# congliuUvA/Clifford-Group-Equivariant-Simplicial-Message-Passing-Networks

Measured on AMD Instinct MI355X. Metric: simplicial edges/sec (fwd+bwd) on Cl(3,0) 8-ch multivectors; % HBM roofline, higher is better.
Workload: dtype f32; 1 GPU; S1: EGCL layer fwd+bwd, Cl(1, 1, 1), 8 channels, 10000 nodes, 100000 edges/GPU x 1 GPU, aggr=mean, edge_attr 6ch, node_attr 3ch; aggregation=float atomics, launch=hip-graph replay

## Files before the change

clifford-group-equivariant-simplicial-message-passing-networks_amd/csmpn_hip/native.py:

```python
from __future__ import annotations

import ctypes as C
import os

_HERE = os.path.dirname(os.path.abspath(__file__))
LIB_PATH = os.environ.get("CSMPN_LIB") or os.path.join(_HERE, "libcsmpn_hip.so")

ABI_VERSION = 2
MAX_BLOCKS = 4
FLAG_WEIGHTS_PACKED = 1
FLAG_NO_VALIDATE = 2
FLAG_DETERMINISTIC = 4
FLAG_SAVE_STATE = 8
ERR_UNSUPPORTED, ERR_INVALID, ERR_HIP = 1, 2, 3

EXPORTS = (
    "csmpn_metric_supported",
    "csmpn_algebra_tables",
    "csmpn_geometric_product_forward",
    "csmpn_geometric_product_backward",
    "csmpn_cemlp_workspace_bytes",
    "csmpn_cemlp_saved_floats_per_row",
    "csmpn_cemlp_saved_floats",
    "csmpn_cemlp_forward",
# ... 4 lines not shown
    "csmpn_mvsilu_backward",
    "csmpn_mvnorm_forward",
    "csmpn_mvnorm_backward",
    "csmpn_mvlayernorm_forward",
    "csmpn_mvlayernorm_backward",
    "csmpn_wgp_forward",
    "csmpn_wgp_backward",
    "csmpn_csr_workspace_bytes",
    "csmpn_csr_build",
    "csmpn_csr_source_order",
    "csmpn_segment_reduce",
    "csmpn_egcl_edge_forward",
    "csmpn_egcl_edge_backward",
    "csmpn_egcl_node_forward",
    "csmpn_egcl_node_backward",
    "csmpn_simplex_rows",
    "csmpn_embed_cemlp_forward",
    "csmpn_embed_cemlp_backward",
    "csmpn_type_attr_forward",
    "csmpn_type_attr_backward",
    "csmpn_readout_mse_forward",
    "csmpn_readout_mse_backward",
    "csmpn_readout_traj_forward",
    "csmpn_readout_traj_backward",
    "csmpn_last_error",
    "csmpn_last_kernel",
    "csmpn_abi_version",
    "csmpn_build_target",
)

# ... 61 lines not shown
    sig("csmpn_mvlayernorm_backward", C.c_int, [fp, C.c_int, vp, vp, vp, i64, i32, vp, vp, vp])
    sig("csmpn_wgp_forward", C.c_int, [fp, C.c_int, vp, vp, vp, i64, i32, vp, vp])
    sig("csmpn_wgp_backward", C.c_int, [fp, C.c_int, vp, vp, vp, vp, i64, i32, vp, vp, vp, vp])
    sig("csmpn_csr_workspace_bytes", sz, [i64, i64])
    sig("csmpn_csr_build", C.c_int, [vp, i64, i64, vp, vp, vp, vp, vp, vp, sz, u32, vp])
    sig("csmpn_csr_source_order", C.c_int, [vp, i64, i64, vp, vp, vp, sz, vp])
    sig("csmpn_segment_reduce", C.c_int, [vp, i64, i64, vp, vp, vp, vp, vp, i32, vp])
    sig("csmpn_egcl_edge_forward", C.c_int,
        [fp, C.c_int, bp, C.c_int, vp, i32, vp, i32, vp, vp, vp, i64, i64, vp, vp, vp, sz, u32, vp])
    sig("csmpn_egcl_edge_backward", C.c_int,
        [fp, C.c_int, bp, bg, C.c_int, vp, i32, vp, i32, vp, vp, vp, i64, i64, vp, vp, vp, vp, vp, sz, u32, vp])
    sig("csmpn_egcl_node_forward", C.c_int,
        [fp, C.c_int, bp, C.c_int, vp, i32, vp, i32, vp, i32, vp, i32, i32, i64, vp, vp, vp, sz, u32, vp])
    sig("csmpn_egcl_node_backward", C.c_int,
        [fp, C.c_int, bp, bg, C.c_int, vp, i32, vp, i32, vp, i32, vp, i32, i32, i64, vp, vp, vp, vp, vp, vp, sz, u32, vp])
    sig("csmpn_simplex_rows", C.c_int, [C.c_int, C.POINTER(VertexBlock), C.c_int, vp, i64, i32, i64, vp, vp])
    sig("csmpn_embed_cemlp_forward", C.c_int, [fp, C.c_int, bp, C.c_int, vp, i64, i32, vp, i32, i32, i64, vp, vp, vp, sz, u32, vp])
    sig("csmpn_embed_cemlp_backward", C.c_int, [fp, C.c_int, bp, bg, C.c_int, vp, i64, i32, vp, i32, i32, i64, vp, vp, vp, sz, u32, vp])
    sig("csmpn_type_attr_forward", C.c_int, [C.c_int, vp, i32, i32, vp, i64, vp, vp, i64, vp, vp, vp])
    sig("csmpn_type_attr_backward", C.c_int, [C.c_int, i32, i32, vp, i64, vp, vp, i64, vp, vp, vp, vp])
    sig("csmpn_readout_mse_forward", C.c_int, [C.c_int, vp, vp, i32, vp, i64, i32, vp, i64, vp, vp, vp, vp, vp])
    sig("csmpn_readout_mse_backward", C.c_int, [C.c_int, vp, i32, i64, i32, vp, i64, vp, vp, vp])
    sig("csmpn_readout_traj_forward", C.c_int, [C.c_int, vp, i32, vp, i64, vp, i32, i32, vp, vp, vp, vp, i64, vp, vp, vp, vp])
    sig("csmpn_readout_traj_backward", C.c_int,
        [C.c_int, vp, i32, i64, vp, vp, i64, vp, i32, i32, vp, vp, vp, vp, vp, vp, vp, vp, vp, vp, vp])
    sig("csmpn_last_error", C.c_char_p, [])
    sig("csmpn_last_kernel", C.c_char_p, [])
    sig("csmpn_abi_version", C.c_int, [])
    sig("csmpn_build_target", C.c_char_p, [])
    return lib
# ... 25 lines not shown
```

clifford-group-equivariant-simplicial-message-passing-networks_amd/csmpn_hip/ops.py:

```python
from __future__ import annotations

import ctypes as C
import os
import warnings
from typing import List, Optional, Sequence

import torch

from . import native
from .native import BlockGrads, BlockParams, PARAM_FIELDS, check

NP = len(PARAM_FIELDS)


def _stream(device) -> int:
    return torch.cuda.current_stream(device).cuda_stream


def _on_device_of(arg_index):
    import functools

    def deco(fn):
        @functools.wraps(fn)
        def wrapped(*args, **kwargs):
# ... 505 lines not shown
            rc = native.lib().csmpn_egcl_edge_backward(
                e.metric_arr, e.n, e.params, e.grads, e.nblk, h.data_ptr(), spec.C, _ptr(edge_attr), spec.A,
                csr.perm.data_ptr(), csr.src.data_ptr(), csr.dst.data_ptr(), csr.n_edges, N, g_agg.data_ptr(),
                rows.data_ptr(), _ptr(g_ea), _ptr(saved), ws.data_ptr(), ws.numel(),
                flags | native.FLAG_DETERMINISTIC, _stream(dev))
            if not (det == "soft" and _soft_fallback(rc)):
                check(rc)
                segment_reduce(rows, gh, add=(csr.row_ptr, None), sub=csr.source_order())
                return g_ea, views
        check(native.lib().csmpn_egcl_edge_backward(
            e.metric_arr, e.n, e.params, e.grads, e.nblk, h.data_ptr(), spec.C, _ptr(edge_attr), spec.A,
            csr.perm.data_ptr(), csr.src.data_ptr(), csr.dst.data_ptr(), csr.n_edges, N, g_agg.data_ptr(),
            gh.data_ptr(), _ptr(g_ea), _ptr(saved), ws.data_ptr(), ws.numel(), flags, _stream(dev)))
        return g_ea, views


_SAVE_STATE = os.environ.get("CSMPN_SAVE_STATE", "1") not in ("0", "")


def _check_egcl_inputs(spec, csr, h, edge_attr, node_attr, n_edges):
    D = spec.edge.D
    if h.dim() != 3 or h.shape[1] != spec.C or h.shape[2] != D:
        raise RuntimeError(f"h must be [N, {spec.C}, {D}], got {tuple(h.shape)}")
    if (edge_attr is None) != (spec.A == 0) or (node_attr is None) != (spec.T == 0):
        raise RuntimeError("edge_attr/node_attr presence does not match edge_attr_features/node_attr_features")
    if edge_attr is not None and tuple(edge_attr.shape) != (n_edges, spec.A, D):
        raise RuntimeError(f"edge_attr must be [{n_edges}, {spec.A}, {D}], got {tuple(edge_attr.shape)}")
    if node_attr is not None and tuple(node_attr.shape) != (h.shape[0], spec.T, D):
        raise RuntimeError(f"node_attr must be [{h.shape[0]}, {spec.T}, {D}], got {tuple(node_attr.shape)}")

# ... 41 lines not shown
        pos = 2
        edge_attr = node_attr = None
        if ctx.has_ea:
            edge_attr = saved[pos]; pos += 1
        if ctx.has_na:
            node_attr = saved[pos]; pos += 1
        it = iter(saved[pos:])
        params = [next(it) if m else None for m in ctx.mask]
        ne = spec.edge.nblk * NP
        pe, pn = params[:ne], params[ne:]
        gout = gout.contiguous()
        gfe, gfn = ctx.gflats if ctx.gflats is not None else (None, None)
        ctx.gflats = None
        refs = ctx.param_refs
        fuse = _fusable(refs, h.device)
        gh, g_agg, g_na, views_n = HipBackend.node_backward(spec, csr.deg, h, agg, node_attr, pn, gout,
                                                            ctx.needs_input_grad[2], ctx.st_n, gfn,
                                                            fused_into=refs[ne:] if fuse else None)
        g_ea, views_e = HipBackend.edge_backward(spec, csr, h, edge_attr, pe, g_agg, gh, ctx.needs_input_grad[1],
                                                 ctx.st_e, gfe, fused_into=refs[:ne] if fuse else None)
        return (gh, g_ea, g_na, None, None, *views_e, *views_n)


def egcl_apply(h, edge_attr, node_attr, spec: EgclSpec, csr: Csr, params):
    return _EgclFn.apply(h, edge_attr, node_attr, spec, csr, *params)




class _GpFn(torch.autograd.Function):
# ... 448 lines not shown
```

clifford-group-equivariant-simplicial-message-passing-networks_amd/csrc/capi.hip:

```cpp
#include <mutex>
#include <hip/hip_runtime.h>

#include <cstdarg>
#include <cstdio>
#include <cstdlib>
#include <cstring>
#include <vector>

#include "plan.hpp"

using namespace csmpn;

thread_local char g_csmpn_err[512] = "";

int csmpn_fail(int code, const char* fmt, ...) {
    va_list ap;
    va_start(ap, fmt);
    vsnprintf(g_csmpn_err, sizeof(g_csmpn_err), fmt, ap);
    va_end(ap);
    return code;
}


namespace csmpn {
// ... 258 lines not shown
                            float* save_inputs, void* workspace, size_t workspace_bytes, uint32_t flags, void* stream) {
    const AlgId id = alg_id(metric, n);
    if (id == ALG_NONE) return fail(CSMPN_ERR_UNSUPPORTED, "metric not supported by the HIP path");
    RowIO io;
    int rc = edge_io(blocks, h, channels, edge_attr, attr_channels, perm, src_sorted, dst_sorted, E, flags, io);
    if (rc) return rc;
    Plan plan;
    if ((rc = make_plan(id, blocks, nullptr, n_blocks, workspace, workspace_bytes, false, blocks[n_blocks - 1].out_features << n, false,
                        E, plan, (flags & CSMPN_FLAG_DETERMINISTIC) != 0))) return rc;
    const bool need_pack = !(flags & CSMPN_FLAG_WEIGHTS_PACKED);
    io.agg = agg; io.save = save_inputs;
    (void)N;
    return run_rows(plan, MODE_EDGE, false, io, (hipStream_t)stream, need_pack);
}

int csmpn_egcl_edge_backward(const float* metric, int n, const csmpn_block_params* blocks,
                             const csmpn_block_grads* grads, int n_blocks, const float* h, int32_t channels,
                             const float* edge_attr, int32_t attr_channels, const int32_t* perm,
                             const int32_t* src_sorted, const int32_t* dst_sorted, int64_t E, int64_t N,
                             const float* g_agg, float* gh, float* g_edge_attr, const float* saved_inputs, void* workspace,
                             size_t workspace_bytes, uint32_t flags, void* stream) {
    const AlgId id = alg_id(metric, n);
    if (id == ALG_NONE) return fail(CSMPN_ERR_UNSUPPORTED, "metric not supported by the HIP path");
    RowIO io;
    int rc = edge_io(blocks, h, channels, edge_attr, attr_channels, perm, src_sorted, dst_sorted, E, flags, io);
    if (rc) return rc;
    Plan plan;
    if ((rc = make_plan(id, blocks, grads, n_blocks, workspace, workspace_bytes, true, 0, saved_inputs != nullptr, E, plan,
                        (flags & CSMPN_FLAG_DETERMINISTIC) != 0))) return rc;
    const bool need_pack = true;
    io.gy = g_agg; io.gx[0] = gh; io.gx[1] = g_edge_attr; io.saved = saved_inputs;
    (void)N;
    return run_rows(plan, MODE_EDGE, true, io, (hipStream_t)stream, need_pack, (flags & CSMPN_FLAG_WEIGHTS_PACKED) != 0);
}

static int node_io(const csmpn_block_params* blocks, int n_blocks, const float* h, int channels, const float* agg,
                   int agg_channels, const float* node_attr, int attr_channels, const int32_t* in_degree,
                   int mean_aggr, int residual, int64_t N, RowIO& io) {
    if (attr_channels > 0 && !node_attr) return fail(CSMPN_ERR_INVALID, "node_attr is null");
    if (channels + agg_channels + attr_channels != blocks[0].in_features)
        return fail(CSMPN_ERR_INVALID, "node model in_features %d != %d + %d + %d", blocks[0].in_features, channels,
                    agg_channels, attr_channels);
    if (residual && blocks[n_blocks - 1].out_features != channels)
        return fail(CSMPN_ERR_INVALID, "residual needs out_features == channels");
    if (mean_aggr && !in_degree) return fail(CSMPN_ERR_INVALID, "in_degree is null");
    memset(&io, 0, sizeof(io));
    io.rows = N; io.nseg = attr_channels > 0 ? 3 : 2;
    io.seg[0].a = h; io.seg[0].ch = channels; io.seg[0].off = 0;
// ... 11 lines not shown
    if (id == ALG_NONE) return fail(CSMPN_ERR_UNSUPPORTED, "metric not supported by the HIP path");
    RowIO io;
    int rc = node_io(blocks, n_blocks, h, channels, agg, agg_channels, node_attr, attr_channels, in_degree, mean_aggr,
                     residual, N, io);
    if (rc) return rc;
    Plan plan;
    if ((rc = make_plan(id, blocks, nullptr, n_blocks, workspace, workspace_bytes, false, 0, false, N, plan,
                        (flags & CSMPN_FLAG_DETERMINISTIC) != 0))) return rc;
    const bool need_pack = !(flags & CSMPN_FLAG_WEIGHTS_PACKED);
    io.y = out; io.resid = residual ? h : nullptr; io.save = save_inputs;
    io.row_store = (flags & CSMPN_FLAG_DETERMINISTIC) ? 1 : 0;
    io.save_state = (flags & CSMPN_FLAG_SAVE_STATE) ? 1 : 0;
    return run_rows(plan, MODE_NODE, false, io, (hipStream_t)stream, need_pack);
}

int csmpn_egcl_node_backward(const float* metric, int n, const csmpn_block_params* blocks,
                             const csmpn_block_grads* grads, int n_blocks, const float* h, int32_t channels,
                             const float* agg, int32_t agg_channels, const float* node_attr, int32_t attr_channels,
                             const int32_t* in_degree, int32_t mean_aggr, int32_t residual, int64_t N,
                             const float* g_out, float* gh, float* g_agg, float* g_node_attr, const float* saved_inputs, void* workspace,
                             size_t workspace_bytes, uint32_t flags, void* stream) {
    const AlgId id = alg_id(metric, n);
    if (id == ALG_NONE) return fail(CSMPN_ERR_UNSUPPORTED, "metric not supported by the HIP path");
    RowIO io;
    int rc = node_io(blocks, n_blocks, h, channels, agg, agg_channels, node_attr, attr_channels, in_degree, mean_aggr,
                     residual, N, io);
    if (rc) return rc;
    Plan plan;
    if ((rc = make_plan(id, blocks, grads, n_blocks, workspace, workspace_bytes, true, 0, saved_inputs != nullptr, N, plan,
                        (flags & CSMPN_FLAG_DETERMINISTIC) != 0))) return rc;
    const bool need_pack = true;
    io.gy = g_out; io.gx[0] = gh; io.gx[1] = g_agg; io.gx[2] = g_node_attr;
    io.resid_bwd = residual ? 1 : 0; io.saved = saved_inputs;
    io.row_store = (flags & CSMPN_FLAG_DETERMINISTIC) ? 1 : 0;
    io.save_state = (flags & CSMPN_FLAG_SAVE_STATE) ? 1 : 0;
    return run_rows(plan, MODE_NODE, true, io, (hipStream_t)stream, need_pack, (flags & CSMPN_FLAG_WEIGHTS_PACKED) != 0);
}

}
```

clifford-group-equivariant-simplicial-message-passing-networks_amd/csrc/cemlp_cl.hpp:

```cpp
#pragma once
#include "cemlp_lane.hpp"

namespace csmpn {

constexpr int kClWaves = 4;
constexpr int kClSliceCap = 512;
constexpr int kClParStride = 36;

#define CL_LDS_ORDER() do { asm volatile("" ::: "memory"); __builtin_amdgcn_wave_barrier(); asm volatile("" ::: "memory"); } while (0)

struct ClStamp {
#ifdef CSMPN_STAMPS
    static constexpr int kSlots = 24;
    unsigned long long t0, acc[kSlots];
    CSMPN_DEV explicit ClStamp(int) {
#pragma unroll
        for (int i = 0; i < kSlots; ++i) acc[i] = 0;
        t0 = __builtin_amdgcn_s_memtime();
    }
    CSMPN_DEV void operator()(int id) {
        __builtin_amdgcn_sched_barrier(0);
        const unsigned long long t1 = __builtin_amdgcn_s_memtime();
        acc[id] += t1 - t0;
        t0 = t1;
// ... 1116 lines not shown
        ClStage<ALG, C, TB1, true> st1;
        st0.load(Cd.b[0], threadIdx.x, dir);
        if constexpr (NBLK > 1) st1.load(Cd.b[1], threadIdx.x, dir);
        st0.store(smem, threadIdx.x);
        if constexpr (NBLK > 1) st1.store(smem + TB0::total, threadIdx.x);
    }
    __syncthreads();
    stamp(0);
    const long ntiles = (io.rows + ClMap<C>::RPW - 1) / ClMap<C>::RPW;
    if (ntiles <= (long)gridDim.x * kClWaves) cl_bwd_blocks<ALG, C, MODE, NBLK, NA, SAVES, true>(io, smem, T0, req, stamp);
    else cl_bwd_blocks<ALG, C, MODE, NBLK, NA, SAVES, false>(io, smem, T0, req, stamp);
    stamp.flush(io.stamps, threadIdx.x & 63);
}

template <class ALG, int C, int I0, int NBLK>
__global__ void __launch_bounds__(256) cl_reduce_kernel(const DevCemlp Cd, const float* part, int nslices, int slice_cap) {
    constexpr int G = ALG::G;
    using P0 = ClPart<ALG, C, I0>;
    using P1 = ClPart<ALG, C, C>;
    constexpr int total = P0::total + (NBLK > 1 ? P1::total : 0);
    __shared__ float red[16][17];
    const int j = threadIdx.x & 15, w = threadIdx.x >> 4;
    int e = blockIdx.x * 16 + j;
    const bool live = e < total;
    if (!live) e = 0;
    const int k = (NBLK > 1 && e >= P0::total) ? 1 : 0;
    const int len = k == 0 ? P0::total : P1::total;
    const float* p = part + (k == 0 ? 0 : (size_t)slice_cap * P0::total);
    if (k == 1) e -= P0::total;
    float s = 0.f;
    for (int s0 = w; s0 < nslices; s0 += 256) {
        float v[16];
#pragma unroll
        for (int i = 0; i < 16; ++i) {
            const int sl = s0 + 16 * i;
            v[i] = sl < nslices ? p[(size_t)sl * len + e] : 0.f;
        }
#pragma unroll
// ... 12 lines not shown
    if (f < nW1) dst = B.gW1 + f;
    else if ((f -= nW1) < nWC) dst = B.gWR + f;
    else if ((f -= nWC) < nWC) dst = B.gWL + f;
    else {
        f -= nWC;
        if (f < P0::qsa) dst = B.has_b1 ? B.gb1 + f : nullptr;
        else if (f < P0::qsb) dst = B.gsa + (f - P0::qsa);
        else if (f < P0::qw) dst = B.gsb + (f - P0::qsb);
        else if (f < P0::qan) dst = B.gw + (f - P0::qw);
        else if (f < P0::qbL) dst = B.gan + (f - P0::qan);
        else if (f < P0::qla) dst = B.gbL + (f - P0::qbL);
        else dst = B.gla + (f - P0::qla);
    }
    if (dst) *dst += s;
}

}
```

clifford-group-equivariant-simplicial-message-passing-networks_amd/csrc/cemlp_device.hpp:

```cpp
#pragma once
#include <hip/hip_runtime.h>

#include "algebra.hpp"

namespace csmpn {

typedef float f4 __attribute__((ext_vector_type(4)));

#define CSMPN_DEV __device__ __forceinline__
#define CSMPN_PHASE() __builtin_amdgcn_sched_barrier(0)

constexpr float kInvSqrt2 = 0.70710678118654752440f;
constexpr float kEps = 1e-6f;
constexpr float kSmooth = 1e-16f;


struct DevBlock {
    int I, O;
    int KKi, KKo;
    int NTi, NTo;
    int CPi, CPo;
    int has_b1;
    int lds_goff;
    int lds_woff;
// ... 36 lines not shown

struct RowIO {
    long rows;
    int nseg;
    int pad_;
    Seg seg[3];
    float* y;
    const float* resid;
    float* agg;
    const int* dst;
    const int* src;
    const int* perm;
    const float* gy;
    float* gx[3];
    int resid_bwd;
    int pad2_;
    float* save;
    const float* saved;
    unsigned long long* stamps;
    float* rl_partials;
    int row_store;
    int save_state;
    const float* tabs;
    float* handover;
    float* slices;
    const int* emb_verts;
    int emb_nperm, emb_nv, emb_k, emb_nrows;
};

enum { VAR_WAVE = 0, VAR_GROUP = 1, VAR_GROUP_NM = 2, VAR_GLOBAL = 3 };
template <int VAR> constexpr bool kVarBarrier = VAR != VAR_WAVE;
// ... 746 lines not shown
```

clifford-group-equivariant-simplicial-message-passing-networks_amd/csrc/cl_inst.inc:

```
#include "cemlp_cl.hpp"
#include "launch_unit.hpp"

namespace csmpn {
namespace {
using ALG_T = Alg<CSMPN_ALG_N, CSMPN_ALG_NEG>;
static_assert(kClSliceCap == kClMaxBwdGroups, "the host sizes the partial buffer for the slices the kernels lay it out for");

template <int C, int MODE, int NBLK, int NA>
constexpr size_t cl_part_floats() {
    return ClPart<ALG_T, C, ClTab<C, MODE, NA, 0, true>::I>::total + (NBLK > 1 ? ClPart<ALG_T, C, C>::total : 0);
}

template <int C, int MODE, int NBLK, int NA>
hipError_t cl_launch(bool bwd, bool, unsigned grid, hipStream_t st, const DevCemlp& Cd, const RowIO& io, float*) {
    if (!bwd) {
        constexpr size_t lds = cl_fwd_lds_bytes<ALG_T, C, MODE, NBLK, NA>();
        return launch_kernel<cemlp_cl_fwd_kernel<ALG_T, C, MODE, NBLK, NA>>(grid, 64 * kClWaves, lds, st, Cd, io);
    }
    if (grid > (unsigned)kClSliceCap) return hipErrorInvalidValue;
    constexpr size_t lds = cl_bwd_lds_bytes<ALG_T, C, MODE, NBLK, NA>();
    static_assert(2 * lds <= 160 * 1024, "two workgroups per CU");
    const hipError_t e0 = io.save_state ? launch_kernel<cemlp_cl_bwd_kernel<ALG_T, C, MODE, NBLK, NA, true>>(grid, 64 * kClWaves, lds, st, Cd, io)
                                        : launch_kernel<cemlp_cl_bwd_kernel<ALG_T, C, MODE, NBLK, NA, false>>(grid, 64 * kClWaves, lds, st, Cd, io);
    if (e0 != hipSuccess) return e0;
    constexpr int I0 = ClTab<C, MODE, NA, 0, true>::I;
    constexpr int total = (int)cl_part_floats<C, MODE, NBLK, NA>();
    return launch_kernel<cl_reduce_kernel<ALG_T, C, I0, NBLK>>((total + 15) / 16, 256, 0, st, Cd, (const float*)io.rl_partials, (int)grid,
                                                              (int)kClSliceCap);
}

template <int C, int MODE, int NBLK, int NA>
constexpr LaneEntry cl_entry() { return {{MODE, NBLK, C, NA}, 0, cl_part_floats<C, MODE, NBLK, NA>(), cl_launch<C, MODE, NBLK, NA>}; }
constexpr LaneEntry kShapes[] = {cl_entry<8, MODE_EDGE, 2, 6>(), cl_entry<8, MODE_NODE, 2, 3>()};
}

const LaneUnit& CSMPN_CAT(cemlp_cl_, CSMPN_ALG_TAG)() { return LaneUnitOf<kShapes>::unit; }
}
```

clifford-group-equivariant-simplicial-message-passing-networks_amd/csrc/dispatch.hip:

```cpp
#include <atomic>
#include <cstdio>

#include "plan.hpp"

namespace csmpn {

namespace {
LaneShape shape_of(int mode, int nblk, int ch, int i0) {
    return LaneShape{mode, nblk, ch, mode == MODE_EDGE ? i0 - ch : (mode == MODE_NODE ? i0 - 2 * ch : i0)};
}
size_t pq_region_bytes(int nblk, int ch, int i0) {
    size_t best = 0;
    for (int mode : {MODE_EDGE, MODE_NODE, MODE_PLAIN}) {
        const LaneShape s = shape_of(mode, nblk, ch, i0);
        const size_t tf = cemlp_pq_n3().table_floats(s);
        if (!tf) continue;
        const size_t b = (tf + cemlp_pq_n3().slice_floats(s) * kPqGridCap) * sizeof(float) + 1024;
        best = b > best ? b : best;
    }
    return best;
}
size_t egcl_slice_floats(const LaneUnit& u, int nblk, int ch, int i0) {
    const size_t e = u.slice_floats(shape_of(MODE_EDGE, nblk, ch, i0)), n = u.slice_floats(shape_of(MODE_NODE, nblk, ch, i0));
    return n > e ? n : e;
// ... 291 lines not shown
    if (F.debug_fields == kI0) snprintf(shape, sizeof(shape), "i0=%d", x.S.i0);
    else snprintf(shape, sizeof(shape), "channels=%d %s=%d", x.S.ch, F.debug_fields == kChannelsAttr ? "attr" : "i0",
                  F.debug_fields == kChannelsAttr ? x.S.na : x.S.i0);
    fprintf(stderr, "[csmpn] %s mode=%d bwd=%d %s grid=%u rows=%ld\n", F.name, x.mode, (int)x.bwd, shape, grid, rows);
}

Launch make_launch(const Plan& plan, int mode, bool bwd, bool tables_ready, const RowIO& io, float* handover) {
    return Launch{plan, alg_ops(plan.id), mode, bwd, tables_ready, stage_shape(plan.C, mode, io), handover};
}
}

bool plw_serves(const Plan& plan, int mode, bool bwd, const RowIO& io) {
    return plw_eligible(make_launch(plan, mode, bwd, false, io, nullptr), io);
}

int run_rows(const Plan& plan, int mode, bool bwd, const RowIO& io_in, hipStream_t st, bool need_pack, bool tables_ready) {
    if (io_in.rows <= 0) return CSMPN_OK;
    const AlgOps& A = alg_ops(plan.id);
    RowIO io = io_in;
    io.stamps = g_stamps;
    const SavedLayout SL = saved_layout(A.n, plan.blocks, plan.C.nblk, io.rows, io.save_state ? CSMPN_FLAG_SAVE_STATE : 0);
    if (!SL.state_ch) io.save_state = 0;
    float* const handover = io.saved ? const_cast<float*>(io.saved) + SL.handover_off : nullptr;
    const Launch x = make_launch(plan, mode, bwd, tables_ready, io, handover);
    for (const Family& F : kFamilies) {
        if (!F.eligible(x, io)) continue;
        const unsigned grid = F.grid(x, io.rows);
        float* tabs = nullptr;
        const int rc = F.regions(x, io, &tabs);
        if (rc) return rc;
        if (sw().debug) debug_line(F, x, grid, io.rows);
        bool handled = false;
        HIP_TRY(F.unit(A)->launch(lane_shape(x), bwd, !(bwd && tables_ready), grid, st, plan.C, io, tabs, &handled));
        if (handled) {
            F.kernel_label(x, io);
            return CSMPN_OK;
        }
    }
    if (A.D == 32 && bwd && mode != MODE_PLAIN && io.rows >= 4096 && !sw().quiet) {
        static std::atomic<bool> warned{false};
        if (!warned.exchange(true))
            fprintf(stderr, "[csmpn] note: Cl(5,0) / Cl(4,1) layer with %d channels runs on the general row-tile kernels (slow path: "
                            "their backward spills registers). The parity-lane kernels serve two-block EGCL layers of 8, 16, 24, 28 "
                            "or 32 channels. (CSMPN_QUIET=1 silences this note.)\n", plan.C.b[0].O);
    }
    if (io.row_store && !plan.det_general)
        return fail(CSMPN_ERR_UNSUPPORTED,
                    "CSMPN_FLAG_DETERMINISTIC: this shape is served neither by the lane kernels (Cl(3,0) 8 / 16 channels, "
                    "Cl(5,0) / Cl(4,1) 8 / 16 / 24 / 28 / 32 channels; two blocks with saved block inputs) nor by the deterministic "
// ... 56 lines not shown
```

clifford-group-equivariant-simplicial-message-passing-networks_amd/csrc/launch.hpp:

```cpp
#pragma once
#include <hip/hip_runtime.h>

#include "cemlp_device.hpp"

namespace csmpn {
constexpr int kMaxLdsBytes = 160 * 1024;

#define CSMPN_DECLARE_ALG(tag)                                                                                  \
    bool has_h2_##tag();                                                                                        \
    bool has_ps_##tag();                                                                                        \
    hipError_t launch_cemlp_ps_##tag(int mode, bool bwd, unsigned grid, unsigned block, size_t lds,            \
                                     hipStream_t st, const DevCemlp& C, const RowIO& io);                      \
    hipError_t launch_cemlp_##tag(int mode, int var, int h, bool bwd, unsigned grid, unsigned block, size_t lds,   \
                                  hipStream_t st, const DevCemlp& C, const RowIO& io);                          \
    hipError_t launch_cemlp_wide_##tag(int mode, bool bwd, unsigned grid, unsigned block, size_t lds, hipStream_t st, \
                                       const DevCemlp& C, const RowIO& io);                                    \
    hipError_t launch_gp_##tag(bool bwd, const float* a, const float* b, const float* gout, float* out,        \
                               float* ga, float* gb, long rows, hipStream_t st);

CSMPN_DECLARE_ALG(n2)
CSMPN_DECLARE_ALG(n3)
CSMPN_DECLARE_ALG(n4)
CSMPN_DECLARE_ALG(n5)
CSMPN_DECLARE_ALG(n5m)
CSMPN_DECLARE_ALG(n4m)

struct LaneShape { int mode, nblk, channels, attr; };
struct LaneUnit {
    size_t (*table_floats)(const LaneShape&);
    size_t (*slice_floats)(const LaneShape&);
    hipError_t (*launch)(const LaneShape&, bool bwd, bool pack, unsigned grid, hipStream_t st, const DevCemlp& C, const RowIO& io,
                         float* tabs, bool* handled);
};
inline bool serves(const LaneUnit& u, const LaneShape& s) { return u.table_floats(s) != 0 || u.slice_floats(s) != 0; }
#define CSMPN_DECLARE_LANE_UNIT(family, tag) const LaneUnit& cemlp_##family##_##tag();

constexpr int kClMaxFwdGroups = 1024;
constexpr int kClMaxBwdGroups = 512;
CSMPN_DECLARE_LANE_UNIT(cl, n3)

constexpr int kCmMaxFwdGroups = 768;
constexpr int kCmMaxBwdGroups = 256;
CSMPN_DECLARE_LANE_UNIT(cm, n3)

constexpr int kPlMaxBwdGroups = 256;
CSMPN_DECLARE_LANE_UNIT(pl, n5)
CSMPN_DECLARE_LANE_UNIT(pl, n5m)
// ... 27 lines not shown
```

clifford-group-equivariant-simplicial-message-passing-networks_amd/csrc/launch_unit.hpp:

```cpp
#pragma once
#include <atomic>

#include "launch.hpp"

#define CSMPN_CAT2(a, b) a##b
#define CSMPN_CAT(a, b) CSMPN_CAT2(a, b)

namespace csmpn {
constexpr int kMaxDevices = 64;

template <auto Kern, class... Args>
hipError_t launch_kernel(unsigned grid, unsigned block, size_t lds, hipStream_t st, const Args&... args) {
    if (lds > 64 * 1024) {
        static std::atomic<size_t> lds_enabled[kMaxDevices];
        int dev = 0;
        if (hipGetDevice(&dev) != hipSuccess || dev < 0 || dev >= kMaxDevices) dev = 0;
        if (lds > lds_enabled[dev].load(std::memory_order_relaxed)) {
            hipError_t e = hipFuncSetAttribute(reinterpret_cast<const void*>(Kern), hipFuncAttributeMaxDynamicSharedMemorySize, (int)lds);
            if (e != hipSuccess) return e;
            lds_enabled[dev].store(lds, std::memory_order_relaxed);
        }
    }
    hipLaunchKernelGGL(Kern, dim3(grid), dim3(block), lds, st, args...);
    return hipGetLastError();
}

struct LaneEntry {
    LaneShape shape;
    size_t table_floats, slice_floats;
    hipError_t (*launch)(bool bwd, bool pack, unsigned grid, hipStream_t st, const DevCemlp& C, const RowIO& io, float* tabs);
};

template <const auto& Table>
struct LaneUnitOf {
    static const LaneEntry* find(const LaneShape& s) {
        for (const LaneEntry& e : Table)
            if (e.shape.mode == s.mode && e.shape.nblk == s.nblk && e.shape.channels == s.channels && e.shape.attr == s.attr) return &e;
        return nullptr;
    }
    static size_t table_floats(const LaneShape& s) {
        const LaneEntry* e = find(s);
        return e ? e->table_floats : 0;
    }
    static size_t slice_floats(const LaneShape& s) {
        const LaneEntry* e = find(s);
        return e ? e->slice_floats : 0;
    }
    static hipError_t launch(const LaneShape& s, bool bwd, bool pack, unsigned grid, hipStream_t st, const DevCemlp& C, const RowIO& io,
                             float* tabs, bool* handled) {
        const LaneEntry* e = find(s);
        *handled = e != nullptr;
        return e ? e->launch(bwd, pack, grid, st, C, io, tabs) : hipSuccess;
    }
    static constexpr LaneUnit unit{table_floats, slice_floats, launch};
};
}
```

clifford-group-equivariant-simplicial-message-passing-networks_amd/csrc/plan.hpp:

```cpp
#pragma once
#include <hip/hip_runtime.h>

#include <cstddef>

#include "../../include/csmpn_hip.h"
#include "capi_common.hpp"
#include "cemlp_kernel.hpp"
#include "launch.hpp"

#define fail csmpn_fail

#define HIP_TRY(expr)                                                                         \
    do {                                                                                      \
        hipError_t e_ = (expr);                                                               \
        if (e_ != hipSuccess) return fail(CSMPN_ERR_HIP, "%s: %s", #expr, hipGetErrorString(e_)); \
    } while (0)

namespace csmpn {

inline int cdiv(int a, int b) { return (a + b - 1) / b; }
inline int rup(int a, int b) { return cdiv(a, b) * b; }

struct Switches {
    bool no_cl;
// ... 81 lines not shown
};
size_t det_slice_bytes(int n, const csmpn_block_params* blocks, int nblk);
int det_slices(const Plan& plan, bool required, DetSlices& S);
int det_launch_begin(const Plan& plan, const DetSlices& S, long grid, DevCemlp& Cd, hipStream_t st);
int det_reduce(const Plan& plan, const DetSlices& S, long grid, hipStream_t st);

struct SavedLayout {
    size_t inputs_ch, handover_ch, state_ch;
    size_t handover_off, state_off, total;
};
SavedLayout saved_layout(int n, const csmpn_block_params* blocks, int nblk, int64_t rows, uint32_t flags);
bool pq_plain_shape(int n, const csmpn_block_params* blocks, int nblk);
bool general_phased_shape(int n, const csmpn_block_params* blocks, int nblk);
size_t family_tail_bytes(int n, const csmpn_block_params* blocks, int nblk);

int run_rows(const Plan& plan, int mode, bool bwd, const RowIO& io_in, hipStream_t st, bool need_pack, bool tables_ready = false);
bool plw_serves(const Plan& plan, int mode, bool bwd, const RowIO& io);

}
```

include/csmpn_hip.h:

```cpp
#ifndef CSMPN_HIP_H
#define CSMPN_HIP_H

#include <stddef.h>
#include <stdint.h>

#ifdef __cplusplus
extern "C" {
#endif

#define CSMPN_MAX_BLOCKS 4
#define CSMPN_OK 0
#define CSMPN_ERR_UNSUPPORTED 1
#define CSMPN_ERR_INVALID 2
#define CSMPN_ERR_HIP 3

#define CSMPN_FLAG_NO_VALIDATE 2u
#define CSMPN_FLAG_WEIGHTS_PACKED 1u

#define CSMPN_FLAG_DETERMINISTIC 4u
#define CSMPN_FLAG_SAVE_STATE 8u

typedef struct csmpn_block_params {
    int32_t in_features;
    int32_t out_features;
// ... 96 lines not shown
                             const float* saved_inputs, void* workspace, size_t workspace_bytes, uint32_t flags, void* stream);

int csmpn_egcl_node_forward(const float* metric_host, int n, const csmpn_block_params* blocks, int n_blocks,
                            const float* h, int32_t channels, const float* agg, int32_t agg_channels,
                            const float* node_attr, int32_t attr_channels, const int32_t* in_degree,
                            int32_t mean_aggr, int32_t residual, int64_t n_nodes, float* out,
                            float* save_inputs, void* workspace, size_t workspace_bytes, uint32_t flags, void* stream);

int csmpn_egcl_node_backward(const float* metric_host, int n, const csmpn_block_params* blocks,
                             const csmpn_block_grads* grads, int n_blocks, const float* h, int32_t channels,
                             const float* agg, int32_t agg_channels, const float* node_attr,
                             int32_t attr_channels, const int32_t* in_degree, int32_t mean_aggr,
                             int32_t residual, int64_t n_nodes, const float* g_out, float* gh, float* g_agg,
                             float* g_node_attr, const float* saved_inputs, void* workspace, size_t workspace_bytes, uint32_t flags, void* stream);

typedef struct csmpn_vertex_block {
    const float* data;
    int32_t channels;
    int32_t grade;
} csmpn_vertex_block;
int csmpn_simplex_rows(int n, const csmpn_vertex_block* blocks, int n_blocks, const int64_t* verts, int64_t n_rows,
                       int32_t verts_per_row, int64_t n_feature_rows, float* out, void* stream);

int csmpn_embed_cemlp_forward(const float* metric_host, int n, const csmpn_block_params* blocks, int n_blocks,
                              const float* vertex_feat, int64_t n_vertex_rows, int32_t channels_per_vertex, const int32_t* verts,
                              int32_t verts_per_row, int32_t n_orders, int64_t n_rows, float* out, float* save_inputs,
                              void* workspace, size_t workspace_bytes, uint32_t flags, void* stream);
int csmpn_embed_cemlp_backward(const float* metric_host, int n, const csmpn_block_params* blocks, const csmpn_block_grads* grads,
                               int n_blocks, const float* vertex_feat, int64_t n_vertex_rows, int32_t channels_per_vertex,
                               const int32_t* verts, int32_t verts_per_row, int32_t n_orders, int64_t n_rows, const float* g_out,
// ... 36 lines not shown
```

Baseline: 582.4 million edges/s.

## Fuse EGCL layer backward and merge node/edge weight-gradient slice reductions

Adds a single csmpn_egcl_backward entry point that runs the node backward and then the edge backward in one call. The per-slice weight-gradient reduction of each stage is deferred, and both are summed in one combined cl_reduce2 kernel launch. The goal is to drop one reduction kernel launch and some Python/ctypes dispatch overhead per layer backward. It adds a new ABI entry and only applies in non-deterministic mode when the two workspaces do not overlap.

```diff
diff --git a/clifford-group-equivariant-simplicial-message-passing-networks_amd/csmpn_hip/native.py b/clifford-group-equivariant-simplicial-message-passing-networks_amd/csmpn_hip/native.py
--- a/clifford-group-equivariant-simplicial-message-passing-networks_amd/csmpn_hip/native.py
+++ b/clifford-group-equivariant-simplicial-message-passing-networks_amd/csmpn_hip/native.py
@@ -42,6 +42,7 @@
     "csmpn_egcl_edge_backward",
     "csmpn_egcl_node_forward",
     "csmpn_egcl_node_backward",
+    "csmpn_egcl_backward",
     "csmpn_simplex_rows",
     "csmpn_embed_cemlp_forward",
     "csmpn_embed_cemlp_backward",
@@ -133,6 +134,9 @@
         [fp, C.c_int, bp, C.c_int, vp, i32, vp, i32, vp, i32, vp, i32, i32, i64, vp, vp, vp, sz, u32, vp])
     sig("csmpn_egcl_node_backward", C.c_int,
         [fp, C.c_int, bp, bg, C.c_int, vp, i32, vp, i32, vp, i32, vp, i32, i32, i64, vp, vp, vp, vp, vp, vp, sz, u32, vp])
+    sig("csmpn_egcl_backward", C.c_int,
+        [fp, C.c_int, bp, bg, C.c_int, bp, bg, C.c_int, vp, i32, vp, i32, vp, i32, vp, i32, vp, vp, vp, vp, i32, i32, i64, i64,
+         vp, vp, vp, vp, vp, vp, vp, vp, sz, u32, vp, vp, sz, u32, vp])
     sig("csmpn_simplex_rows", C.c_int, [C.c_int, C.POINTER(VertexBlock), C.c_int, vp, i64, i32, i64, vp, vp])
     sig("csmpn_embed_cemlp_forward", C.c_int, [fp, C.c_int, bp, C.c_int, vp, i64, i32, vp, i32, i32, i64, vp, vp, vp, sz, u32, vp])
     sig("csmpn_embed_cemlp_backward", C.c_int, [fp, C.c_int, bp, bg, C.c_int, vp, i64, i32, vp, i32, i32, i64, vp, vp, vp, sz, u32, vp])
diff --git a/clifford-group-equivariant-simplicial-message-passing-networks_amd/csmpn_hip/ops.py b/clifford-group-equivariant-simplicial-message-passing-networks_amd/csmpn_hip/ops.py
--- a/clifford-group-equivariant-simplicial-message-passing-networks_amd/csmpn_hip/ops.py
+++ b/clifford-group-equivariant-simplicial-message-passing-networks_amd/csmpn_hip/ops.py
@@ -543,6 +543,38 @@
             gh.data_ptr(), _ptr(g_ea), _ptr(saved), ws.data_ptr(), ws.numel(), flags, _stream(dev)))
         return g_ea, views
 
+    @staticmethod
+    @_on_device_of(2)
+    def layer_backward(spec, csr, h, agg, edge_attr, node_attr, pe, pn, gout, want_gea, want_gna, state_e=None, state_n=None,
+                       gflat_e=None, gflat_n=None, fused_e=None, fused_n=None):
+        e, nd = spec.edge, spec.node
+        e.bind(pe)
+        nd.bind(pn)
+        N, D, dev = h.shape[0], nd.D, h.device
+        _fe, views_e = e.new_grads(pe, dev, gflat_e, fused_into=fused_e)
+        _fn, views_n = nd.new_grads(pn, dev, gflat_n, fused_into=fused_n)
+        gh = torch.empty_like(h)
+        g_agg = torch.empty(N, spec.O, D, dtype=torch.float32, device=dev)
+        g_na = torch.empty_like(node_attr) if (node_attr is not None and want_gna) else None
+        g_ea = torch.empty_like(edge_attr) if (edge_attr is not None and want_gea) else None
+
+        def stage(binding, state):
+            ws, saved = state if state is not None else (binding.workspace(dev), None)
+            flags = native.FLAG_WEIGHTS_PACKED if state is not None else 0
+            if getattr(saved, "csmpn_save_state", False):
+                flags |= native.FLAG_SAVE_STATE
+            return ws, saved, flags
+
+        ws_e, saved_e, fl_e = stage(e, state_e)
+        ws_n, saved_n, fl_n = stage(nd, state_n)
+        check(native.lib().csmpn_egcl_backward(
+            e.metric_arr, e.n, e.params, e.grads, e.nblk, nd.params, nd.grads, nd.nblk, h.data_ptr(), spec.C,
+            agg.data_ptr(), spec.O, _ptr(edge_attr), spec.A, _ptr(node_attr), spec.T, csr.perm.data_ptr(),
+            csr.src.data_ptr(), csr.dst.data_ptr(), csr.deg.data_ptr(), spec.mean, spec.residual, csr.n_edges, N,
+            gout.data_ptr(), gh.data_ptr(), g_agg.data_ptr(), _ptr(g_ea), _ptr(g_na), None, _ptr(saved_e),
+            ws_e.data_ptr(), ws_e.numel(), fl_e, _ptr(saved_n), ws_n.data_ptr(), ws_n.numel(), fl_n, _stream(dev)))
+        return gh, g_ea, g_na, views_e, views_n
+
 
 _SAVE_STATE = os.environ.get("CSMPN_SAVE_STATE", "1") not in ("0", "")
 
@@ -614,6 +646,11 @@
         ctx.gflats = None
         refs = ctx.param_refs
         fuse = _fusable(refs, h.device)
+        if isinstance(csr, Csr) and not deterministic_request():
+            gh, g_ea, g_na, views_e, views_n = HipBackend.layer_backward(
+                spec, csr, h, agg, edge_attr, node_attr, pe, pn, gout, ctx.needs_input_grad[1], ctx.needs_input_grad[2],
+                ctx.st_e, ctx.st_n, gfe, gfn, refs[:ne] if fuse else None, refs[ne:] if fuse else None)
+            return (gh, g_ea, g_na, None, None, *views_e, *views_n)
         gh, g_agg, g_na, views_n = HipBackend.node_backward(spec, csr.deg, h, agg, node_attr, pn, gout,
                                                             ctx.needs_input_grad[2], ctx.st_n, gfn,
                                                             fused_into=refs[ne:] if fuse else None)
diff --git a/clifford-group-equivariant-simplicial-message-passing-networks_amd/csrc/capi.hip b/clifford-group-equivariant-simplicial-message-passing-networks_amd/csrc/capi.hip
--- a/clifford-group-equivariant-simplicial-message-passing-networks_amd/csrc/capi.hip
+++ b/clifford-group-equivariant-simplicial-message-passing-networks_amd/csrc/capi.hip
@@ -296,24 +296,34 @@
     return run_rows(plan, MODE_EDGE, false, io, (hipStream_t)stream, need_pack);
 }
 
+static int edge_backward(const float* metric, int n, const csmpn_block_params* blocks,
+                         const csmpn_block_grads* grads, int n_blocks, const float* h, int32_t channels,
+                         const float* edge_attr, int32_t attr_channels, const int32_t* perm,
+                         const int32_t* src_sorted, const int32_t* dst_sorted, int64_t E, int64_t N,
+                         const float* g_agg, float* gh, float* g_edge_attr, const float* saved_inputs, void* workspace,
+                         size_t workspace_bytes, uint32_t flags, void* stream, SliceSet* deferred) {
+    const AlgId id = alg_id(metric, n);
+    if (id == ALG_NONE) return fail(CSMPN_ERR_UNSUPPORTED, "metric not supported by the HIP path");
+    RowIO io;
+    int rc = edge_io(blocks, h, channels, edge_attr, attr_channels, perm, src_sorted, dst_sorted, E, flags, io);
+    if (rc) return rc;
+    Plan plan;
+    if ((rc = make_plan(id, blocks, grads, n_blocks, workspace, workspace_bytes, true, 0, saved_inputs != nullptr, E, plan,
+                        (flags & CSMPN_FLAG_DETERMINISTIC) != 0))) return rc;
+    const bool need_pack = true;
+    io.gy = g_agg; io.gx[0] = gh; io.gx[1] = g_edge_attr; io.saved = saved_inputs;
+    (void)N;
+    return run_rows(plan, MODE_EDGE, true, io, (hipStream_t)stream, need_pack, (flags & CSMPN_FLAG_WEIGHTS_PACKED) != 0, deferred);
+}
+
 int csmpn_egcl_edge_backward(const float* metric, int n, const csmpn_block_params* blocks,
                              const csmpn_block_grads* grads, int n_blocks, const float* h, int32_t channels,
                              const float* edge_attr, int32_t attr_channels, const int32_t* perm,
                              const int32_t* src_sorted, const int32_t* dst_sorted, int64_t E, int64_t N,
                              const float* g_agg, float* gh, float* g_edge_attr, const float* saved_inputs, void* workspace,
                              size_t workspace_bytes, uint32_t flags, void* stream) {
-    const AlgId id = alg_id(metric, n);
-    if (id == ALG_NONE) return fail(CSMPN_ERR_UNSUPPORTED, "metric not supported by the HIP path");
-    RowIO io;
-    int rc = edge_io(blocks, h, channels, edge_attr, attr_channels, perm, src_sorted, dst_sorted, E, flags, io);
-    if (rc) return rc;
-    Plan plan;
-    if ((rc = make_plan(id, blocks, grads, n_blocks, workspace, workspace_bytes, true, 0, saved_inputs != nullptr, E, plan,
-                        (flags & CSMPN_FLAG_DETERMINISTIC) != 0))) return rc;
-    const bool need_pack = true;
-    io.gy = g_agg; io.gx[0] = gh; io.gx[1] = g_edge_attr; io.saved = saved_inputs;
-    (void)N;
-    return run_rows(plan, MODE_EDGE, true, io, (hipStream_t)stream, need_pack, (flags & CSMPN_FLAG_WEIGHTS_PACKED) != 0);
+    return edge_backward(metric, n, blocks, grads, n_blocks, h, channels, edge_attr, attr_channels, perm, src_sorted, dst_sorted, E, N,
+                         g_agg, gh, g_edge_attr, saved_inputs, workspace, workspace_bytes, flags, stream, nullptr);
 }
 
 static int node_io(const csmpn_block_params* blocks, int n_blocks, const float* h, int channels, const float* agg,
@@ -355,12 +365,12 @@
     return run_rows(plan, MODE_NODE, false, io, (hipStream_t)stream, need_pack);
 }
 
-int csmpn_egcl_node_backward(const float* metric, int n, const csmpn_block_params* blocks,
-                             const csmpn_block_grads* grads, int n_blocks, const float* h, int32_t channels,
-                             const float* agg, int32_t agg_channels, const float* node_attr, int32_t attr_channels,
-                             const int32_t* in_degree, int32_t mean_aggr, int32_t residual, int64_t N,
-                             const float* g_out, float* gh, float* g_agg, float* g_node_attr, const float* saved_inputs, void* workspace,
-                             size_t workspace_bytes, uint32_t flags, void* stream) {
+static int node_backward(const float* metric, int n, const csmpn_block_params* blocks,
+                         const csmpn_block_grads* grads, int n_blocks, const float* h, int32_t channels,
+                         const float* agg, int32_t agg_channels, const float* node_attr, int32_t attr_channels,
+                         const int32_t* in_degree, int32_t mean_aggr, int32_t residual, int64_t N,
+                         const float* g_out, float* gh, float* g_agg, float* g_node_attr, const float* saved_inputs, void* workspace,
+                         size_t workspace_bytes, uint32_t flags, void* stream, SliceSet* deferred) {
     const AlgId id = alg_id(metric, n);
     if (id == ALG_NONE) return fail(CSMPN_ERR_UNSUPPORTED, "metric not supported by the HIP path");
     RowIO io;
@@ -375,7 +385,49 @@
     io.resid_bwd = residual ? 1 : 0; io.saved = saved_inputs;
     io.row_store = (flags & CSMPN_FLAG_DETERMINISTIC) ? 1 : 0;
     io.save_state = (flags & CSMPN_FLAG_SAVE_STATE) ? 1 : 0;
-    return run_rows(plan, MODE_NODE, true, io, (hipStream_t)stream, need_pack, (flags & CSMPN_FLAG_WEIGHTS_PACKED) != 0);
-}
-
-}
+    return run_rows(plan, MODE_NODE, true, io, (hipStream_t)stream, need_pack, (flags & CSMPN_FLAG_WEIGHTS_PACKED) != 0, deferred);
+}
+
+int csmpn_egcl_node_backward(const float* metric, int n, const csmpn_block_params* blocks,
+                             const csmpn_block_grads* grads, int n_blocks, const float* h, int32_t channels,
+                             const float* agg, int32_t agg_channels, const float* node_attr, int32_t attr_channels,
+                             const int32_t* in_degree, int32_t mean_aggr, int32_t residual, int64_t N,
+                             const float* g_out, float* gh, float* g_agg, float* g_node_attr, const float* saved_inputs, void* workspace,
+                             size_t workspace_bytes, uint32_t flags, void* stream) {
+    return node_backward(metric, n, blocks, grads, n_blocks, h, channels, agg, agg_channels, node_attr, attr_channels, in_degree, mean_aggr,
+                         residual, N, g_out, gh, g_agg, g_node_attr, saved_inputs, workspace, workspace_bytes, flags, stream, nullptr);
+}
+
+int csmpn_egcl_backward(const float* metric, int n, const csmpn_block_params* edge_blocks, const csmpn_block_grads* edge_grads,
+                        int n_edge_blocks, const csmpn_block_params* node_blocks, const csmpn_block_grads* node_grads,
+                        int n_node_blocks, const float* h, int32_t channels, const float* agg, int32_t agg_channels,
+                        const float* edge_attr, int32_t edge_attr_channels, const float* node_attr, int32_t node_attr_channels,
+                        const int32_t* perm, const int32_t* src_sorted, const int32_t* dst_sorted, const int32_t* in_degree,
+                        int32_t mean_aggr, int32_t residual, int64_t E, int64_t N, const float* g_out, float* gh, float* g_agg,
+                        float* g_edge_attr, float* g_node_attr, float* g_edge_rows, const float* edge_saved, void* edge_workspace,
+                        size_t edge_workspace_bytes, uint32_t edge_flags, const float* node_saved, void* node_workspace,
+                        size_t node_workspace_bytes, uint32_t node_flags, void* stream) {
+    const bool det = ((edge_flags | node_flags) & CSMPN_FLAG_DETERMINISTIC) != 0;
+    if ((edge_flags & CSMPN_FLAG_DETERMINISTIC) && !g_edge_rows)
+        return fail(CSMPN_ERR_INVALID, "CSMPN_FLAG_DETERMINISTIC: g_edge_rows ([E, C, D], csmpn_egcl_edge_backward's gh) is null");
+    const char *we = static_cast<const char*>(edge_workspace), *wn = static_cast<const char*>(node_workspace);
+    const bool apart = we && wn && (we + edge_workspace_bytes <= wn || wn + node_workspace_bytes <= we);
+    SliceSet node_set, edge_set;
+    node_set.unit = edge_set.unit = nullptr;
+    const bool defer = !det && apart;
+    int rc = node_backward(metric, n, node_blocks, node_grads, n_node_blocks, h, channels, agg, agg_channels, node_attr,
+                           node_attr_channels, in_degree, mean_aggr, residual, N, g_out, gh, g_agg, g_node_attr, node_saved,
+                           node_workspace, node_workspace_bytes, node_flags, stream, defer ? &node_set : nullptr);
+    if (rc) return rc;
+    rc = edge_backward(metric, n, edge_blocks, edge_grads, n_edge_blocks, h, channels, edge_attr, edge_attr_channels, perm, src_sorted,
+                       dst_sorted, E, N, g_agg, (edge_flags & CSMPN_FLAG_DETERMINISTIC) ? g_edge_rows : gh, g_edge_attr, edge_saved,
+                       edge_workspace, edge_workspace_bytes, edge_flags, stream, node_set.unit ? &edge_set : nullptr);
+    if (node_set.unit) {
+        const SliceSet* const other = (!rc && edge_set.unit == node_set.unit) ? &edge_set : nullptr;
+        HIP_TRY(node_set.unit->sum_slices(node_set, other, (hipStream_t)stream));
+        if (!rc && edge_set.unit && !other) HIP_TRY(edge_set.unit->sum_slices(edge_set, nullptr, (hipStream_t)stream));
+    }
+    return rc;
+}
+
+}
diff --git a/clifford-group-equivariant-simplicial-message-passing-networks_amd/csrc/cemlp_cl.hpp b/clifford-group-equivariant-simplicial-message-passing-networks_amd/csrc/cemlp_cl.hpp
--- a/clifford-group-equivariant-simplicial-message-passing-networks_amd/csrc/cemlp_cl.hpp
+++ b/clifford-group-equivariant-simplicial-message-passing-networks_amd/csrc/cemlp_cl.hpp
@@ -1154,14 +1154,13 @@
 }
 
 template <class ALG, int C, int I0, int NBLK>
-__global__ void __launch_bounds__(256) cl_reduce_kernel(const DevCemlp Cd, const float* part, int nslices, int slice_cap) {
+CSMPN_DEV void cl_reduce_group(const DevCemlp& Cd, const float* part, int nslices, int slice_cap, int group, float (*red)[17]) {
     constexpr int G = ALG::G;
     using P0 = ClPart<ALG, C, I0>;
     using P1 = ClPart<ALG, C, C>;
     constexpr int total = P0::total + (NBLK > 1 ? P1::total : 0);
-    __shared__ float red[16][17];
     const int j = threadIdx.x & 15, w = threadIdx.x >> 4;
-    int e = blockIdx.x * 16 + j;
+    int e = group * 16 + j;
     const bool live = e < total;
     if (!live) e = 0;
     const int k = (NBLK > 1 && e >= P0::total) ? 1 : 0;
@@ -1204,5 +1203,20 @@
     }
     if (dst) *dst += s;
 }
-
-}
+template <class ALG, int C, int I0, int NBLK>
+constexpr int cl_reduce_groups() { return (ClPart<ALG, C, I0>::total + (NBLK > 1 ? ClPart<ALG, C, C>::total : 0) + 15) / 16; }
+template <class ALG, int C, int I0, int NBLK>
+__global__ void __launch_bounds__(256) cl_reduce_kernel(const DevCemlp Cd, const float* part, int nslices, int slice_cap) {
+    __shared__ float red[16][17];
+    cl_reduce_group<ALG, C, I0, NBLK>(Cd, part, nslices, slice_cap, blockIdx.x, red);
+}
+template <class ALG, int C, int I0A, int NBLKA, int I0B, int NBLKB>
+__global__ void __launch_bounds__(256) cl_reduce2_kernel(const DevCemlp CdA, const float* partA, int nslicesA, const DevCemlp CdB,
+                                                         const float* partB, int nslicesB, int slice_cap) {
+    __shared__ float red[16][17];
+    constexpr int groupsA = cl_reduce_groups<ALG, C, I0A, NBLKA>();
+    if ((int)blockIdx.x < groupsA) cl_reduce_group<ALG, C, I0A, NBLKA>(CdA, partA, nslicesA, slice_cap, blockIdx.x, red);
+    else cl_reduce_group<ALG, C, I0B, NBLKB>(CdB, partB, nslicesB, slice_cap, (int)blockIdx.x - groupsA, red);
+}
+
+}
diff --git a/clifford-group-equivariant-simplicial-message-passing-networks_amd/csrc/cemlp_device.hpp b/clifford-group-equivariant-simplicial-message-passing-networks_amd/csrc/cemlp_device.hpp
--- a/clifford-group-equivariant-simplicial-message-passing-networks_amd/csrc/cemlp_device.hpp
+++ b/clifford-group-equivariant-simplicial-message-passing-networks_amd/csrc/cemlp_device.hpp
@@ -74,7 +74,7 @@
     const float* gy;
     float* gx[3];
     int resid_bwd;
-    int pad2_;
+    int defer_sum;
     float* save;
     const float* saved;
     unsigned long long* stamps;
diff --git a/clifford-group-equivariant-simplicial-message-passing-networks_amd/csrc/cl_inst.inc b/clifford-group-equivariant-simplicial-message-passing-networks_amd/csrc/cl_inst.inc
--- a/clifford-group-equivariant-simplicial-message-passing-networks_amd/csrc/cl_inst.inc
+++ b/clifford-group-equivariant-simplicial-message-passing-networks_amd/csrc/cl_inst.inc
@@ -12,6 +12,13 @@
 }
 
 template <int C, int MODE, int NBLK, int NA>
+hipError_t cl_sum(hipStream_t st, const DevCemlp& Cd, const float* part, unsigned nslices) {
+    constexpr int I0 = ClTab<C, MODE, NA, 0, true>::I;
+    return launch_kernel<cl_reduce_kernel<ALG_T, C, I0, NBLK>>(cl_reduce_groups<ALG_T, C, I0, NBLK>(), 256, 0, st, Cd, part, (int)nslices,
+                                                              (int)kClSliceCap);
+}
+
+template <int C, int MODE, int NBLK, int NA>
 hipError_t cl_launch(bool bwd, bool, unsigned grid, hipStream_t st, const DevCemlp& Cd, const RowIO& io, float*) {
     if (!bwd) {
         constexpr size_t lds = cl_fwd_lds_bytes<ALG_T, C, MODE, NBLK, NA>();
@@ -22,17 +29,36 @@
     static_assert(2 * lds <= 160 * 1024, "two workgroups per CU");
     const hipError_t e0 = io.save_state ? launch_kernel<cemlp_cl_bwd_kernel<ALG_T, C, MODE, NBLK, NA, true>>(grid, 64 * kClWaves, lds, st, Cd, io)
                                         : launch_kernel<cemlp_cl_bwd_kernel<ALG_T, C, MODE, NBLK, NA, false>>(grid, 64 * kClWaves, lds, st, Cd, io);
-    if (e0 != hipSuccess) return e0;
-    constexpr int I0 = ClTab<C, MODE, NA, 0, true>::I;
-    constexpr int total = (int)cl_part_floats<C, MODE, NBLK, NA>();
-    return launch_kernel<cl_reduce_kernel<ALG_T, C, I0, NBLK>>((total + 15) / 16, 256, 0, st, Cd, (const float*)io.rl_partials, (int)grid,
-                                                              (int)kClSliceCap);
+    if (e0 != hipSuccess || io.defer_sum) return e0;
+    return cl_sum<C, MODE, NBLK, NA>(st, Cd, io.rl_partials, grid);
 }
 
 template <int C, int MODE, int NBLK, int NA>
 constexpr LaneEntry cl_entry() { return {{MODE, NBLK, C, NA}, 0, cl_part_floats<C, MODE, NBLK, NA>(), cl_launch<C, MODE, NBLK, NA>}; }
 constexpr LaneEntry kShapes[] = {cl_entry<8, MODE_EDGE, 2, 6>(), cl_entry<8, MODE_NODE, 2, 3>()};
+
+bool same_shape(const LaneShape& s, const LaneShape& t) {
+    return s.mode == t.mode && s.nblk == t.nblk && s.channels == t.channels && s.attr == t.attr;
+}
+hipError_t cl_sum_slices(const SliceSet& a, const SliceSet* b, hipStream_t st) {
+    constexpr LaneShape edge = kShapes[0].shape, node = kShapes[1].shape;
+    if (b && same_shape(a.shape, edge) && same_shape(b->shape, node)) return cl_sum_slices(*b, &a, st);
+    if (b && same_shape(a.shape, node) && same_shape(b->shape, edge)) {
+        constexpr int IN = ClTab<8, MODE_NODE, 3, 0, true>::I, IE = ClTab<8, MODE_EDGE, 6, 0, true>::I;
+        constexpr unsigned groups = cl_reduce_groups<ALG_T, 8, IN, 2>() + cl_reduce_groups<ALG_T, 8, IE, 2>();
+        return launch_kernel<cl_reduce2_kernel<ALG_T, 8, IN, 2, IE, 2>>(groups, 256, 0, st, a.C, a.part, (int)a.nslices, b->C, b->part,
+                                                                         (int)b->nslices, (int)kClSliceCap);
+    }
+    for (const SliceSet* s : {&a, b}) {
+        if (!s) continue;
+        hipError_t e = hipErrorInvalidValue;
+        if (same_shape(s->shape, edge)) e = cl_sum<8, MODE_EDGE, 2, 6>(st, s->C, s->part, s->nslices);
+        else if (same_shape(s->shape, node)) e = cl_sum<8, MODE_NODE, 2, 3>(st, s->C, s->part, s->nslices);
+        if (e != hipSuccess) return e;
+    }
+    return hipSuccess;
+}
 }
 
-const LaneUnit& CSMPN_CAT(cemlp_cl_, CSMPN_ALG_TAG)() { return LaneUnitOf<kShapes>::unit; }
+const LaneUnit& CSMPN_CAT(cemlp_cl_, CSMPN_ALG_TAG)() { return LaneUnitOf<kShapes, cl_sum_slices>::unit; }
 }
diff --git a/clifford-group-equivariant-simplicial-message-passing-networks_amd/csrc/dispatch.hip b/clifford-group-equivariant-simplicial-message-passing-networks_amd/csrc/dispatch.hip
--- a/clifford-group-equivariant-simplicial-message-passing-networks_amd/csrc/dispatch.hip
+++ b/clifford-group-equivariant-simplicial-message-passing-networks_amd/csrc/dispatch.hip
@@ -329,7 +329,9 @@
     return plw_eligible(make_launch(plan, mode, bwd, false, io, nullptr), io);
 }
 
-int run_rows(const Plan& plan, int mode, bool bwd, const RowIO& io_in, hipStream_t st, bool need_pack, bool tables_ready) {
+int run_rows(const Plan& plan, int mode, bool bwd, const RowIO& io_in, hipStream_t st, bool need_pack, bool tables_ready,
+             SliceSet* deferred) {
+    if (deferred) deferred->unit = nullptr;
     if (io_in.rows <= 0) return CSMPN_OK;
     const AlgOps& A = alg_ops(plan.id);
     RowIO io = io_in;
@@ -346,8 +348,11 @@
         if (rc) return rc;
         if (sw().debug) debug_line(F, x, grid, io.rows);
         bool handled = false;
-        HIP_TRY(F.unit(A)->launch(lane_shape(x), bwd, !(bwd && tables_ready), grid, st, plan.C, io, tabs, &handled));
+        const LaneUnit* const unit = F.unit(A);
+        io.defer_sum = (bwd && deferred && unit->sum_slices && io.rl_partials) ? 1 : 0;
+        HIP_TRY(unit->launch(lane_shape(x), bwd, !(bwd && tables_ready), grid, st, plan.C, io, tabs, &handled));
         if (handled) {
+            if (io.defer_sum) *deferred = SliceSet{unit, lane_shape(x), plan.C, io.rl_partials, grid};
             F.kernel_label(x, io);
             return CSMPN_OK;
         }
diff --git a/clifford-group-equivariant-simplicial-message-passing-networks_amd/csrc/launch.hpp b/clifford-group-equivariant-simplicial-message-passing-networks_amd/csrc/launch.hpp
--- a/clifford-group-equivariant-simplicial-message-passing-networks_amd/csrc/launch.hpp
+++ b/clifford-group-equivariant-simplicial-message-passing-networks_amd/csrc/launch.hpp
@@ -26,11 +26,20 @@
 CSMPN_DECLARE_ALG(n4m)
 
 struct LaneShape { int mode, nblk, channels, attr; };
+struct LaneUnit;
+struct SliceSet {
+    const LaneUnit* unit;
+    LaneShape shape;
+    DevCemlp C;
+    const float* part;
+    unsigned nslices;
+};
 struct LaneUnit {
     size_t (*table_floats)(const LaneShape&);
     size_t (*slice_floats)(const LaneShape&);
     hipError_t (*launch)(const LaneShape&, bool bwd, bool pack, unsigned grid, hipStream_t st, const DevCemlp& C, const RowIO& io,
                          float* tabs, bool* handled);
+    hipError_t (*sum_slices)(const SliceSet& a, const SliceSet* b, hipStream_t st);
 };
 inline bool serves(const LaneUnit& u, const LaneShape& s) { return u.table_floats(s) != 0 || u.slice_floats(s) != 0; }
 #define CSMPN_DECLARE_LANE_UNIT(family, tag) const LaneUnit& cemlp_##family##_##tag();
diff --git a/clifford-group-equivariant-simplicial-message-passing-networks_amd/csrc/launch_unit.hpp b/clifford-group-equivariant-simplicial-message-passing-networks_amd/csrc/launch_unit.hpp
--- a/clifford-group-equivariant-simplicial-message-passing-networks_amd/csrc/launch_unit.hpp
+++ b/clifford-group-equivariant-simplicial-message-passing-networks_amd/csrc/launch_unit.hpp
@@ -31,7 +31,7 @@
     hipError_t (*launch)(bool bwd, bool pack, unsigned grid, hipStream_t st, const DevCemlp& C, const RowIO& io, float* tabs);
 };
 
-template <const auto& Table>
+template <const auto& Table, hipError_t (*SumSlices)(const SliceSet&, const SliceSet*, hipStream_t) = nullptr>
 struct LaneUnitOf {
     static const LaneEntry* find(const LaneShape& s) {
         for (const LaneEntry& e : Table)
@@ -52,6 +52,6 @@
         *handled = e != nullptr;
         return e ? e->launch(bwd, pack, grid, st, C, io, tabs) : hipSuccess;
     }
-    static constexpr LaneUnit unit{table_floats, slice_floats, launch};
+    static constexpr LaneUnit unit{table_floats, slice_floats, launch, SumSlices};
 };
 }
diff --git a/clifford-group-equivariant-simplicial-message-passing-networks_amd/csrc/plan.hpp b/clifford-group-equivariant-simplicial-message-passing-networks_amd/csrc/plan.hpp
--- a/clifford-group-equivariant-simplicial-message-passing-networks_amd/csrc/plan.hpp
+++ b/clifford-group-equivariant-simplicial-message-passing-networks_amd/csrc/plan.hpp
@@ -119,7 +119,8 @@
 bool general_phased_shape(int n, const csmpn_block_params* blocks, int nblk);
 size_t family_tail_bytes(int n, const csmpn_block_params* blocks, int nblk);
 
-int run_rows(const Plan& plan, int mode, bool bwd, const RowIO& io_in, hipStream_t st, bool need_pack, bool tables_ready = false);
+int run_rows(const Plan& plan, int mode, bool bwd, const RowIO& io_in, hipStream_t st, bool need_pack, bool tables_ready = false,
+             SliceSet* deferred = nullptr);
 bool plw_serves(const Plan& plan, int mode, bool bwd, const RowIO& io);
 
 }
diff --git a/include/csmpn_hip.h b/include/csmpn_hip.h
--- a/include/csmpn_hip.h
+++ b/include/csmpn_hip.h
@@ -134,6 +134,17 @@
                              int32_t residual, int64_t n_nodes, const float* g_out, float* gh, float* g_agg,
                              float* g_node_attr, const float* saved_inputs, void* workspace, size_t workspace_bytes, uint32_t flags, void* stream);
 
+int csmpn_egcl_backward(const float* metric_host, int n, const csmpn_block_params* edge_blocks,
+                        const csmpn_block_grads* edge_grads, int n_edge_blocks, const csmpn_block_params* node_blocks,
+                        const csmpn_block_grads* node_grads, int n_node_blocks, const float* h, int32_t channels,
+                        const float* agg, int32_t agg_channels, const float* edge_attr, int32_t edge_attr_channels,
+                        const float* node_attr, int32_t node_attr_channels, const int32_t* perm, const int32_t* src_sorted,
+                        const int32_t* dst_sorted, const int32_t* in_degree, int32_t mean_aggr, int32_t residual,
+                        int64_t n_edges, int64_t n_nodes, const float* g_out, float* gh, float* g_agg, float* g_edge_attr,
+                        float* g_node_attr, float* g_edge_rows, const float* edge_saved_inputs, void* edge_workspace,
+                        size_t edge_workspace_bytes, uint32_t edge_flags, const float* node_saved_inputs, void* node_workspace,
+                        size_t node_workspace_bytes, uint32_t node_flags, void* stream);
+
 typedef struct csmpn_vertex_block {
     const float* data;
     int32_t channels;
```

Result: faster. 592.9 million edges/s (median of 6 runs) (+1.8%).
